# luo-yining/CFDBench

Hardware: NVIDIA H100
Metric: fno_rollout_steps_per_sec (higher is better)
Workload: dtype bf16

## Files before the change

### cfdbench_b200/csrc/fno_project_tc.cu

```cuda
#include "fno_common.cuh"
#include "tc_common.cuh"

namespace fno {

constexpr int kPtWG = 4;
constexpr int kPtThreads = 128 * kPtWG;
constexpr int kPtM = kW;
constexpr uint32_t kPtLboA = (kPtM / 8) * 128;
constexpr uint32_t kPtLboB = (kProj / 8) * 128;
constexpr int kPtTilesPerSample = kH;
constexpr int kPtReps = kPtM * (kC / 4) / 128;

struct PtSmem {
  alignas(128) float w_hi[kProj * kC];
  alignas(128) float w_lo[kProj * kC];
  alignas(128) float a_hi[kPtWG][kPtM * kC];
  alignas(128) float a_lo[kPtWG][kPtM * kC];
  alignas(16) float4 w2q[kProj / 2];
  alignas(16) float2 b1p[kProj / 2];
};

template <typename TAct>
struct PtRegs {
  TAct v[kPtReps][4];
};

template <typename TAct>
__device__ __forceinline__ void pt_prefetch(PtRegs<TAct>& r, const TAct* __restrict__ a, int tile, int t) {
  const int b = tile / kPtTilesPerSample, p0 = (tile % kPtTilesPerSample) * kPtM;
#pragma unroll
  for (int rep = 0; rep < kPtReps; ++rep) {
    const int task = rep * 128 + t;
    const int m = task & (kPtM - 1), kq = task >> 6;
    const TAct* src = a + (static_cast<size_t>(b) * kC + 4 * kq) * kHW + p0 + m;
#pragma unroll
    for (int c = 0; c < 4; ++c) r.v[rep][c] = __ldg(src + static_cast<size_t>(c) * kHW);
  }
}

__device__ __forceinline__ float pt_to_float(float v) { return v; }
__device__ __forceinline__ float pt_to_float(__nv_bfloat16 v) { return __bfloat162float(v); }

template <typename TAct>
__device__ __forceinline__ void pt_split_store(const PtRegs<TAct>& r, float* a_hi, float* a_lo, int t) {
#pragma unroll
  for (int rep = 0; rep < kPtReps; ++rep) {
    const int task = rep * 128 + t;
    const int m = task & (kPtM - 1), kq = task >> 6;
    float hi[4], lo[4];
#pragma unroll
    for (int c = 0; c < 4; ++c) {
      const float x = pt_to_float(r.v[rep][c]);
      if constexpr (sizeof(TAct) == 4) tc::split_tf32(x, hi[c], lo[c]);
      else hi[c] = x;
    }
    const uint32_t off = tc::kmajor_offset(m, 4 * kq, kPtM) / 4;
    *reinterpret_cast<float4*>(a_hi + off) = make_float4(hi[0], hi[1], hi[2], hi[3]);
    if constexpr (sizeof(TAct) == 4) *reinterpret_cast<float4*>(a_lo + off) = make_float4(lo[0], lo[1], lo[2], lo[3]);
  }
}

template <typename TAct>
__global__ void __launch_bounds__(kPtThreads, 1)
    project_tc_kernel(const TAct* __restrict__ a, const float* __restrict__ w1, const float* __restrict__ b1,
                      const float* __restrict__ w2, const float* __restrict__ b2, const float* __restrict__ mask,
                      float* __restrict__ preds, int n_tiles) {
  constexpr bool kBf16 = sizeof(TAct) == 2;
  extern __shared__ __align__(1024) unsigned char smem_raw[];
  PtSmem& sm = *reinterpret_cast<PtSmem*>(smem_raw);
  const int tid = threadIdx.x, lane = tid & 31;
  const int wg = tc::warp_index_uniform() >> 2, t = tid & 127, wq = (tid >> 5) & 3;

  for (int e = tid; e < kProj * kC; e += kPtThreads) {
    const int j = e / kC, i = e % kC;
    float hi, lo;
    tc::split_tf32(w1[e], hi, lo);
    const uint32_t off = tc::kmajor_offset(j, i, kProj) / 4;
    sm.w_hi[off] = hi;
    sm.w_lo[off] = lo;
  }
  if (tid < kProj / 2) {
    sm.w2q[tid] = make_float4(w2[2 * tid], w2[kProj + 2 * tid], w2[2 * tid + 1], w2[kProj + 2 * tid + 1]);
    sm.b1p[tid] = make_float2(b1[2 * tid], b1[2 * tid + 1]);
  }
  const float b2x = b2[0], b2y = b2[1];
  tc::fence_proxy_async_smem();
  __syncthreads();
  pdl_wait();
  pdl_launch_dependents();

  const int first = blockIdx.x * kPtWG + wg, stride = gridDim.x * kPtWG;
  float* a_hi = sm.a_hi[wg];
  float* a_lo = sm.a_lo[wg];
  PtRegs<TAct> regs;
  if (first < n_tiles) pt_prefetch<TAct>(regs, a, first, t);
  for (int tile = first; tile < n_tiles; tile += stride) {
    pt_split_store<TAct>(regs, a_hi, a_lo, t);
    tc::fence_proxy_async_smem();
    tc::named_barrier(1 + wg, 128);
    if (tile + stride < n_tiles) pt_prefetch<TAct>(regs, a, tile + stride, t);
    float acc[64];
    tc::wg_fence();
    {
      const uint32_t a_s[3] = {tc::smem_addr(a_hi), tc::smem_addr(a_lo), tc::smem_addr(a_hi)};
      const uint32_t b_s[3] = {tc::smem_addr(sm.w_hi), tc::smem_addr(sm.w_hi), tc::smem_addr(sm.w_lo)};
#pragma unroll
      for (int pass = 0; pass < 3; ++pass) {
        if (kBf16 && pass == 1) continue;
#pragma unroll
        for (int ks = 0; ks < kC / 8; ++ks)
          tc::wg_tf32_ss_n128(acc, tc::make_smem_desc(a_s[pass] + ks * 2 * kPtLboA, kPtLboA, 128),
                              tc::make_smem_desc(b_s[pass] + ks * 2 * kPtLboB, kPtLboB, 128), (pass | ks) ? 1u : 0u);
      }
    }
    tc::wg_commit();
    tc::wg_wait<0>();
    tc::wg_fence_acc(acc);
    const int b = tile / kPtTilesPerSample, p0 = (tile % kPtTilesPerSample) * kPtM;
#pragma unroll
    for (int hh = 0; hh < 2; ++hh) {
      float2 out = make_float2(0.f, 0.f);
#pragma unroll
      for (int i0 = 0; i0 < 16; i0 += 8) {
        float2 g[8];
#pragma unroll
        for (int i = 0; i < 8; ++i) {
          const float2 bb = sm.b1p[4 * (i0 + i) + (lane & 3)];
          g[i] = make_float2(acc[4 * (i0 + i) + 2 * hh] + bb.x, acc[4 * (i0 + i) + 2 * hh + 1] + bb.y);
        }
        if constexpr (kBf16) {
          gelu_erf2_deg5_batch<8>(g);
        } else {
#pragma unroll
          for (int i = 0; i < 8; ++i) g[i] = gelu_erf2(g[i]);
        }
#pragma unroll
        for (int i = 0; i < 8; ++i) {
          const float4 wq4 = sm.w2q[4 * (i0 + i) + (lane & 3)];
          out = ffma2(make_float2(g[i].x, g[i].x), make_float2(wq4.x, wq4.y), out);
          out = ffma2(make_float2(g[i].y, g[i].y), make_float2(wq4.z, wq4.w), out);
        }
      }
      out.x += __shfl_xor_sync(0xffffffffu, out.x, 1);
      out.y += __shfl_xor_sync(0xffffffffu, out.y, 1);
      out.x += __shfl_xor_sync(0xffffffffu, out.x, 2);
      out.y += __shfl_xor_sync(0xffffffffu, out.y, 2);
      if ((lane & 3) == 0) {
        const int pix = p0 + 16 * wq + (lane >> 2) + 8 * hh;
        const float mk = __ldg(mask + static_cast<size_t>(b) * kHW + pix);
        preds[(static_cast<size_t>(b) * 2 + 0) * kHW + pix] = (b2x + out.x) * mk;
        preds[(static_cast<size_t>(b) * 2 + 1) * kHW + pix] = (b2y + out.y) * mk;
      }
    }
  }
}

template <typename TAct>
cudaError_t launch_project_tc(const void* a, const float* w1, const float* b1, const float* w2, const float* b2,
                              const float* mask, float* preds, int batch, cudaStream_t stream) {
  auto kern = project_tc_kernel<TAct>;
  constexpr size_t smem = sizeof(PtSmem);
  static PerDeviceLaunch pd;
  int n_sm = 0;
  cudaError_t e0 = per_device_setup(kern, smem, pd, &n_sm);
  if (e0 != cudaSuccess) return e0;
  const int n_tiles = batch * kPtTilesPerSample;
  const int want = (n_tiles + kPtWG - 1) / kPtWG;
  const int grid = want < n_sm ? want : n_sm;
  return launch_chained(kern, dim3(grid), dim3(kPtThreads), smem, stream, static_cast<const TAct*>(a), w1, b1, w2, b2,
                        mask, preds, n_tiles);
}
template cudaError_t launch_project_tc<float>(const void*, const float*, const float*, const float*, const float*,
                                              const float*, float*, int, cudaStream_t);
template cudaError_t launch_project_tc<__nv_bfloat16>(const void*, const float*, const float*, const float*,
                                                      const float*, const float*, float*, int, cudaStream_t);

}
```

Baseline: 1315.

## Pair bf16 activation loads, defer prefetch behind MMA, hoist mask loads

For bf16 activations, each thread loads two adjacent pixels as one 32-bit word and unpacks them with shifts into the K-major smem layout, halving load instructions. The next-tile prefetch now runs after the wgmma commit so global loads overlap the tensor-core work, and the mask value is loaded before the wgmma wait. Tile assignment is interleaved across warpgroups (wg*grid + block) rather than contiguous per block. Holding the prefetch registers across the epilogue may raise register pressure, and the paired path is only taken when the pointer is 4-byte aligned.

Result: no change. 1320 (median of 6 runs) (+0.4%).

```diff
diff --git a/cfdbench_b200/csrc/fno_project_tc.cu b/cfdbench_b200/csrc/fno_project_tc.cu
--- a/cfdbench_b200/csrc/fno_project_tc.cu
+++ b/cfdbench_b200/csrc/fno_project_tc.cu
@@ -1,3 +1,5 @@
+#include <type_traits>
+
 #include "fno_common.cuh"
 #include "tc_common.cuh"
 
@@ -20,47 +22,60 @@
   alignas(16) float2 b1p[kProj / 2];
 };
 
-template <typename TAct>
+template <typename TAct, int kVec>
 struct PtRegs {
-  TAct v[kPtReps][4];
+  static_assert(kVec == 1 || sizeof(TAct) == 2, "paired loads are for bf16 activations");
+  static constexpr int kReps = kPtReps / kVec;
+  using Elem = std::conditional_t<kVec == 2, uint32_t, TAct>;
+  Elem v[kReps][4];
 };
 
-template <typename TAct>
-__device__ __forceinline__ void pt_prefetch(PtRegs<TAct>& r, const TAct* __restrict__ a, int tile, int t) {
+template <typename TAct, int kVec>
+__device__ __forceinline__ void pt_prefetch(PtRegs<TAct, kVec>& r, const TAct* __restrict__ a, int tile, int t) {
   const int b = tile / kPtTilesPerSample, p0 = (tile % kPtTilesPerSample) * kPtM;
 #pragma unroll
-  for (int rep = 0; rep < kPtReps; ++rep) {
+  for (int rep = 0; rep < PtRegs<TAct, kVec>::kReps; ++rep) {
     const int task = rep * 128 + t;
-    const int m = task & (kPtM - 1), kq = task >> 6;
+    const int m = kVec * (task & (kPtM / kVec - 1)), kq = task / (kPtM / kVec);
     const TAct* src = a + (static_cast<size_t>(b) * kC + 4 * kq) * kHW + p0 + m;
 #pragma unroll
-    for (int c = 0; c < 4; ++c) r.v[rep][c] = __ldg(src + static_cast<size_t>(c) * kHW);
+    for (int c = 0; c < 4; ++c) {
+      if constexpr (kVec == 2) r.v[rep][c] = __ldg(reinterpret_cast<const unsigned int*>(src + static_cast<size_t>(c) * kHW));
+      else r.v[rep][c] = __ldg(src + static_cast<size_t>(c) * kHW);
+    }
   }
 }
 
 __device__ __forceinline__ float pt_to_float(float v) { return v; }
 __device__ __forceinline__ float pt_to_float(__nv_bfloat16 v) { return __bfloat162float(v); }
 
-template <typename TAct>
-__device__ __forceinline__ void pt_split_store(const PtRegs<TAct>& r, float* a_hi, float* a_lo, int t) {
-#pragma unroll
-  for (int rep = 0; rep < kPtReps; ++rep) {
+template <typename TAct, int kVec>
+__device__ __forceinline__ void pt_split_store(const PtRegs<TAct, kVec>& r, float* a_hi, float* a_lo, int t) {
+#pragma unroll
+  for (int rep = 0; rep < PtRegs<TAct, kVec>::kReps; ++rep) {
     const int task = rep * 128 + t;
-    const int m = task & (kPtM - 1), kq = task >> 6;
-    float hi[4], lo[4];
-#pragma unroll
-    for (int c = 0; c < 4; ++c) {
-      const float x = pt_to_float(r.v[rep][c]);
-      if constexpr (sizeof(TAct) == 4) tc::split_tf32(x, hi[c], lo[c]);
-      else hi[c] = x;
-    }
-    const uint32_t off = tc::kmajor_offset(m, 4 * kq, kPtM) / 4;
-    *reinterpret_cast<float4*>(a_hi + off) = make_float4(hi[0], hi[1], hi[2], hi[3]);
-    if constexpr (sizeof(TAct) == 4) *reinterpret_cast<float4*>(a_lo + off) = make_float4(lo[0], lo[1], lo[2], lo[3]);
-  }
-}
-
-template <typename TAct>
+    const int m0 = kVec * (task & (kPtM / kVec - 1)), kq = task / (kPtM / kVec);
+#pragma unroll
+    for (int e = 0; e < kVec; ++e) {
+      float hi[4], lo[4];
+#pragma unroll
+      for (int c = 0; c < 4; ++c) {
+        if constexpr (kVec == 2) {
+          hi[c] = __uint_as_float(e ? (r.v[rep][c] & 0xffff0000u) : (r.v[rep][c] << 16));
+        } else {
+          const float x = pt_to_float(r.v[rep][c]);
+          if constexpr (sizeof(TAct) == 4) tc::split_tf32(x, hi[c], lo[c]);
+          else hi[c] = x;
+        }
+      }
+      const uint32_t off = tc::kmajor_offset(m0 + e, 4 * kq, kPtM) / 4;
+      *reinterpret_cast<float4*>(a_hi + off) = make_float4(hi[0], hi[1], hi[2], hi[3]);
+      if constexpr (sizeof(TAct) == 4) *reinterpret_cast<float4*>(a_lo + off) = make_float4(lo[0], lo[1], lo[2], lo[3]);
+    }
+  }
+}
+
+template <typename TAct, int kVec>
 __global__ void __launch_bounds__(kPtThreads, 1)
     project_tc_kernel(const TAct* __restrict__ a, const float* __restrict__ w1, const float* __restrict__ b1,
                       const float* __restrict__ w2, const float* __restrict__ b2, const float* __restrict__ mask,
@@ -89,16 +104,15 @@
   pdl_wait();
   pdl_launch_dependents();
 
-  const int first = blockIdx.x * kPtWG + wg, stride = gridDim.x * kPtWG;
+  const int first = wg * gridDim.x + blockIdx.x, stride = gridDim.x * kPtWG;
   float* a_hi = sm.a_hi[wg];
   float* a_lo = sm.a_lo[wg];
-  PtRegs<TAct> regs;
-  if (first < n_tiles) pt_prefetch<TAct>(regs, a, first, t);
+  PtRegs<TAct, kVec> regs;
+  if (first < n_tiles) pt_prefetch<TAct, kVec>(regs, a, first, t);
   for (int tile = first; tile < n_tiles; tile += stride) {
-    pt_split_store<TAct>(regs, a_hi, a_lo, t);
+    pt_split_store<TAct, kVec>(regs, a_hi, a_lo, t);
     tc::fence_proxy_async_smem();
     tc::named_barrier(1 + wg, 128);
-    if (tile + stride < n_tiles) pt_prefetch<TAct>(regs, a, tile + stride, t);
     float acc[64];
     tc::wg_fence();
     {
@@ -114,9 +128,14 @@
       }
     }
     tc::wg_commit();
+    if (tile + stride < n_tiles) pt_prefetch<TAct, kVec>(regs, a, tile + stride, t);
+    const int b = tile / kPtTilesPerSample, p0 = (tile % kPtTilesPerSample) * kPtM;
+    float mk[2];
+#pragma unroll
+    for (int hh = 0; hh < 2; ++hh)
+      mk[hh] = (lane & 3) == 0 ? __ldg(mask + static_cast<size_t>(b) * kHW + p0 + 16 * wq + (lane >> 2) + 8 * hh) : 0.f;
     tc::wg_wait<0>();
     tc::wg_fence_acc(acc);
-    const int b = tile / kPtTilesPerSample, p0 = (tile % kPtTilesPerSample) * kPtM;
 #pragma unroll
     for (int hh = 0; hh < 2; ++hh) {
       float2 out = make_float2(0.f, 0.f);
@@ -147,18 +166,17 @@
       out.y += __shfl_xor_sync(0xffffffffu, out.y, 2);
       if ((lane & 3) == 0) {
         const int pix = p0 + 16 * wq + (lane >> 2) + 8 * hh;
-        const float mk = __ldg(mask + static_cast<size_t>(b) * kHW + pix);
-        preds[(static_cast<size_t>(b) * 2 + 0) * kHW + pix] = (b2x + out.x) * mk;
-        preds[(static_cast<size_t>(b) * 2 + 1) * kHW + pix] = (b2y + out.y) * mk;
-      }
-    }
-  }
-}
-
-template <typename TAct>
-cudaError_t launch_project_tc(const void* a, const float* w1, const float* b1, const float* w2, const float* b2,
-                              const float* mask, float* preds, int batch, cudaStream_t stream) {
-  auto kern = project_tc_kernel<TAct>;
+        preds[(static_cast<size_t>(b) * 2 + 0) * kHW + pix] = (b2x + out.x) * mk[hh];
+        preds[(static_cast<size_t>(b) * 2 + 1) * kHW + pix] = (b2y + out.y) * mk[hh];
+      }
+    }
+  }
+}
+
+template <typename TAct, int kVec>
+cudaError_t launch_project_tc_vec(const TAct* a, const float* w1, const float* b1, const float* w2, const float* b2,
+                                  const float* mask, float* preds, int batch, cudaStream_t stream) {
+  auto kern = project_tc_kernel<TAct, kVec>;
   constexpr size_t smem = sizeof(PtSmem);
   static PerDeviceLaunch pd;
   int n_sm = 0;
@@ -167,8 +185,17 @@
   const int n_tiles = batch * kPtTilesPerSample;
   const int want = (n_tiles + kPtWG - 1) / kPtWG;
   const int grid = want < n_sm ? want : n_sm;
-  return launch_chained(kern, dim3(grid), dim3(kPtThreads), smem, stream, static_cast<const TAct*>(a), w1, b1, w2, b2,
-                        mask, preds, n_tiles);
+  return launch_chained(kern, dim3(grid), dim3(kPtThreads), smem, stream, a, w1, b1, w2, b2, mask, preds, n_tiles);
+}
+
+template <typename TAct>
+cudaError_t launch_project_tc(const void* a, const float* w1, const float* b1, const float* w2, const float* b2,
+                              const float* mask, float* preds, int batch, cudaStream_t stream) {
+  const TAct* act = static_cast<const TAct*>(a);
+  if constexpr (sizeof(TAct) == 2)
+    if ((reinterpret_cast<uintptr_t>(a) & 3u) == 0)
+      return launch_project_tc_vec<TAct, 2>(act, w1, b1, w2, b2, mask, preds, batch, stream);
+  return launch_project_tc_vec<TAct, 1>(act, w1, b1, w2, b2, mask, preds, batch, stream);
 }
 template cudaError_t launch_project_tc<float>(const void*, const float*, const float*, const float*, const float*,
                                               const float*, float*, int, cudaStream_t);
```
